# cvlab-stonybrook/s-volsdf

Measured on AMD Instinct MI355X. Metric: rendered rays/sec (1024-ray batch, 128 samples), higher is better.
Workload: dtype f32 (every product, forward and backward, as three fp16 MFMA products of two-piece fp16 operands with f32 accumulate; activation blocks hold both pieces: float32 accuracy class); 1 GPU; configs[1]: VolOpt.train_step (forward + MVS prior lookup + loss + backward + clip/guard/Adam), train mode, fast=1: 1024 rays/GPU x 128 coarse + 98 composited samples + 2048 eikonal points, 8x256 SDF MLP + 4x256 radiance MLP; mode=train, mlp_precision=fp16x2, launch=eager launches, rays_per_gpu=1024, rays_total=1024

## Files before the change

### include/svolsdf_hip.h

```cpp
#ifndef SVOLSDF_HIP_H
#define SVOLSDF_HIP_H

#include <stddef.h>
#include <stdint.h>

#ifdef __cplusplus
extern "C" {
#endif

int svs_version(void);
const char* svs_last_error_string(void);

int svs_set_deterministic(int on);
int svs_get_deterministic(void);

int svs_rays_from_uv(const float* uv, const float* pose, const float* intrinsics, int n_rays, float* ray_dirs,
                     float* cam_loc, float* depth_scale, void* hip_stream);

int svs_eikonal_points(const float* uniform_points, const float* cam_loc, const float* z_eik, const float* ray_dirs,
                       int n_rays, float* points, void* hip_stream);
int svs_stage_in(const void* pinned_host, void* device, size_t bytes, void* hip_stream);
int svs_split_last(const float* z, int n_rays, int n, float* head, float* last, void* hip_stream);

enum { SVS_MMA_F32 = 0, SVS_MMA_F16X2 = 1, SVS_MMA_F16X2_HALF = 2 };
// ... 55 lines not shown
                   const float* stream, int precision, float* abuf, float* sbar_out, float* absmax, void* hip_stream);
int svs_composite_bg(int n_rays, int n_samples, int n_bg, const float* z, const float* z_max, const float* sdf,
                     const float* rgb, const float* normals, const float* depth_scale, const float* beta_param,
                     float beta_min, const float* z_bg, const float* bg_out0, const float* bg_rgb, const float* bg_depth,
                     float* weights, float* bg_trans, float* bg_weights, float* rgb_values, float* depth_values,
                     float* depth_values_all, float* depth_vals, float* normal_map, void* hip_stream);
int svs_composite_bg_bwd(int n_rays, int n_samples, int n_bg, const float* z, const float* z_max, const float* sdf,
                         const float* rgb, const float* depth_scale, const float* beta_param, float beta_min,
                         const float* z_bg, const float* bg_out0, const float* bg_rgb, const float* d_rgb_values,
                         const float* d_weights, const float* d_depth_values, const float* d_depth_all,
                         const float* bg_depth, float* d_sdf, float* d_rgb,
                         float* d_bg_out0, float* d_bg_rgb, float* d_beta_ray, float* d_beta_param, void* hip_stream);

typedef struct svs_wgrad_job {
  const float *a0, *b0; long long sa0, sb0;
  const float *a1, *b1; long long sa1, sb1;
  const float* b_extra; long long s_extra;
  int n_points, ldw;
  float *dW, *db;
  const float* absmax;
  const float *rec0, *rec1;
} svs_wgrad_job;
int svs_wgrad_multi(const svs_wgrad_job* jobs, int n_jobs, int precision, void* hip_stream);
int svs_wgrad(const float* a0, const float* b0, long long sa0, long long sb0, const float* a1, const float* b1,
              long long sa1, long long sb1, const float* b_extra, long long s_extra, int n_points, int precision,
              const float* absmax, const float* rec0, const float* rec1, float* dW, int ldw, float* db, void* hip_stream);

size_t svs_block_bytes(int n_points, int blocks_per_tile);
size_t svs_rgb_zbuf_bytes(int n_points);
size_t svs_sdf_ubuf_bytes(int n_points);
size_t svs_sdf_gbuf_bytes(int n_points);
int svs_rgb_bwd(int n_points, const float* d_rgb, const float* rgb, const float* rbuf, const float* stream, int precision,
                float* zbuf, float* feat_bar, float* d_normals, float* absmax, void* hip_stream);
int svs_sdf_bwd_a(const float* points, int n_points, const float* cam, int cam_stride, const float* dirs, const float* z,
                  int S, int n_rays, const float* d_grad, const unsigned char* clamp_mask, const float* hbuf,
                  const float* gbuf, const float* stream, int precision, float* ubuf, float* a2buf, float* pebuf,
                  float* absmax, void* hip_stream);
int svs_sdf_bwd_b(int n_points, const float* d_sdf, const unsigned char* clamp_mask, const float* feat_bar,
                  int n_feat_points, const float* hbuf, const float* gbuf, const float* a2buf, const float* ubuf,
                  const float* stream, int precision, float* abuf, float* sbar_out, float* absmax, void* hip_stream);
int svs_lin8_row0_grad(const float* hbuf, const float* ubuf, const float* sbar, int n_points, int precision, float* out257,
                       void* hip_stream);
int svs_unpack_wgrad(const float* dWk, const float* dbk, int ldw, int map, int rows, int cols, int row_off,
                     const float* weight_v, const float* weight_g, const float* row0, float* grad_v, float* grad_g,
                     float* grad_b, void* hip_stream);
typedef struct svs_unpack_job {
// ... 255 lines not shown
```

### s-volsdf_amd/csrc/svs_wgrad.hip

```cpp
#include "svs_common.h"
#include "svs_mlp_layout.h"
#include "svs_ticket.h"
#include "svs_wgrad_maps.h"
#include <cstdlib>
#include <type_traits>

namespace svs {
namespace wgrad {

struct Pair {
  const float* a;
  const float* b;
  size_t stride_a, stride_b;
};

struct Args {
  Pair p[2];
  int n_pairs;
  int n_tiles;
  int n_valid_points;
  const float* b_extra;
  size_t stride_extra;
  float* dW;
  int ldw;
// ... 148 lines not shown
  __builtin_amdgcn_sched_barrier(0);
}
__device__ __forceinline__ unsigned lds_addr(const void* p) {
  return (unsigned)(unsigned long long)SVS_LDS(const void, p);
}

__device__ __forceinline__ void scale_from_absmax(const float* absmax, float& s, float& inv_s) {
  s = 1.0f; inv_s = 1.0f;
  if (!absmax) return;
  int e = (int)((__float_as_uint(*absmax) >> 23) & 0xff);
  e = e < 16 ? 16 : (e > 250 ? 250 : e);
  s = __uint_as_float((unsigned)(268 - e) << 23);
  inv_s = __uint_as_float((unsigned)(e - 14) << 23);
}

struct Job {
  Pair p[2];
  const float* rec[2];
  int n_pairs;
  int n_tiles;
  int n_valid_points;
  int b_tiles;
  int col0;
  float* dW;
  int ldw;
  float* db;
  const float* absmax;
  int wg_begin, wg_count;
  det::Ticket ticket;
};
constexpr int kMaxJobs = 20;
struct MultiArgs { Job job[kMaxJobs]; int n_jobs; int touch; int reverse; };
static_assert(sizeof(MultiArgs) <= 4096, "kernel arguments");

constexpr int kThreadsW = 512;
constexpr int kRT = 2, kCT = 16;
static_assert(maps::plane_reads_ok(kPlane), "transposed reads of the operand planes: bank conflict");
static_assert(maps::narrow_reads_ok(kExtraPiece), "transposed reads of the narrow B image: bank conflict");
static_assert(kPlane % 256 == 0 && kNarrowImg % 256 == 0 && kExtraPiece % 256 == 0 && Ring<true>::kSlotAll % 256 == 0 &&
              Ring<false>::kSlotAll % 256 == 0, "every region the reads are offset by starts on a 256-byte bank row");

typedef const __attribute__((address_space(1))) void* gvoid;

template <bool GP>
__global__ __launch_bounds__(kThreadsW, 1) void wgrad_h2_multi_kernel(MultiArgs ma) {
  typedef Ring<GP> R;
  constexpr int kSlot = R::kSlot, kSlotAll = R::kSlotAll, kRing = R::kRing, kAhead = R::kAhead, kB = R::kB;
  extern __shared__ __attribute__((aligned(16))) unsigned char smem_h2[];
  int jj = 0;
  for (int q = 1; q < ma.n_jobs; ++q) if ((int)blockIdx.x >= ma.job[q].wg_begin) jj = q;
  const Job& a = ma.job[jj];
  const int wg = (int)blockIdx.x - a.wg_begin, nwg = a.wg_count;
  const int tid = threadIdx.x, lane = tid & 63;
  const int wave = __builtin_amdgcn_readfirstlane(tid >> 6);
  const bool narrow = a.b_tiles == 1;
  float s_grad, inv_s;
  scale_from_absmax(a.absmax, s_grad, inv_s);

  f32x4 acc[kRT][kCT];
#pragma unroll
  for (int o = 0; o < kRT; ++o)
#pragma unroll
    for (int i = 0; i < kCT; ++i) acc[o][i] = (f32x4)(0.0f);
  float bsum[kRT];
#pragma unroll
  for (int o = 0; o < kRT; ++o) bsum[o] = 0.0f;

  unsigned char* ring = smem_h2;

  const int rg = lane >> 4;
  const int rd_even = maps::plane_base(0, lane), rd_odd = maps::plane_base(1, lane);
  const int a_off = 1024 * kRT * wave;
  const int rx = maps::narrow_base(lane);
  const int wp = lane & 31, whf = lane >> 5;
  const int wxoff = maps::narrow_at(8 * (wave & 3) + 4 * whf, wp);
  const int n_ct = narrow ? 2 : kCT;

  const bool two_pairs = a.n_pairs == 2;
  const int my_tiles = a.n_tiles > wg ? (a.n_tiles - 1 - wg) / nwg + 1 : 0;
  const int n_items = two_pairs ? 2 * my_tiles : my_tiles;
  const int n_valid = a.n_valid_points;
  const bool has_db = a.db != nullptr;
  const bool rev = ma.reverse != 0;
  const float* const pa0 = a.p[0].a; const float* const pb0 = a.p[0].b;
  const float* const pa1 = a.p[1].a; const float* const pb1 = a.p[1].b;
  const size_t sa0 = a.p[0].stride_a, sb0 = a.p[0].stride_b, sa1 = a.p[1].stride_a, sb1 = a.p[1].stride_b;
  const float* const rec0 = a.rec[0]; const float* const rec1 = a.rec[1];
  const bool has_scale = a.absmax != nullptr;
  auto tile_of = [&](int item) {
    const int k = two_pairs ? item >> 1 : item;
    return rev ? wg + (my_tiles - 1 - k) * nwg : wg + k * nwg;
  };

  auto issue = [&](int item) {
    const int t = tile_of(item), pi = two_pairs ? item & 1 : 0;
    const float* pa = (pi ? pa1 : pa0) + (size_t)t * (pi ? sa1 : sa0);
    const float* pb = (pi ? pb1 : pb0) + (size_t)t * (pi ? sb1 : sb0);
    unsigned char* slot = ring + (item % kRing) * kSlotAll;
#pragma unroll
    for (int j = 0; j < 2 * R::kPlanes; ++j) {
      const int piece = wave + 8 * j;
      __builtin_amdgcn_global_load_lds((gvoid)(reinterpret_cast<const f32x4*>(pa) + piece * 64 + lane),
                                       SVS_LDS(void, slot + piece * 1024), 16, 0, 0);
      if (!narrow)
        __builtin_amdgcn_global_load_lds((gvoid)(reinterpret_cast<const f32x4*>(pb) + piece * 64 + lane),
                                         SVS_LDS(void, slot + kB + piece * 1024), 16, 0, 0);
    }
    if (narrow)
      __builtin_amdgcn_global_load_lds((gvoid)(reinterpret_cast<const f32x4*>(pb) + (wave & 3) * 64 + lane),
                                       SVS_LDS(void, slot + kB + (wave & 3) * 1024), 16, 0, 0);
    if (has_scale)
      __builtin_amdgcn_global_load_lds((gvoid)((pi ? rec1 : rec0) + (size_t)t * 64 + lane),
                                       SVS_LDS(void, slot + kSlot + wave * 256), 4, 0, 0);
  };
  unsigned sink = 0;
  auto touch = [&](int item) {
    const int t = tile_of(item), pi = two_pairs ? item & 1 : 0;
    const Pair& p = a.p[pi];
    constexpr int kLines = R::kPlanes * (kPlane / 128);
    const int nb = narrow ? 32 : kLines;
    const float* q = tid < kLines ? p.a + (size_t)t * p.stride_a + tid * 32
                                  : p.b + (size_t)t * p.stride_b + (tid - kLines) * 32;
    if (tid < kLines + nb) asm volatile("global_load_dword %0, %1, off" : "+v"(sink) : "v"(q) : "memory");
  };
  const int ops = (narrow ? 2 * R::kPlanes + 1 : 4 * R::kPlanes) + (has_scale ? 1 : 0);

  auto stage_factors = [&](int item) {
// ... 50 lines not shown
  };
  for (int item = 0; item < n_items; ++item) {
    const int pi = two_pairs ? item & 1 : 0;
    const bool p0 = pi == 0;
    pre_stage(item);
    asm volatile("s_waitcnt lgkmcnt(0)\n\ts_barrier" ::: "memory");
    if (narrow) {
      stage_narrow(item);
      asm volatile("s_waitcnt lgkmcnt(0)\n\ts_barrier" ::: "memory");
    }
    auto issue_next = [&]() {
      if (item + kAhead < n_items) issue(item + kAhead);
      touched = false;
      if (touching && item + kAhead + 1 < n_items) { touch(item + kAhead + 1); touched = true; }
    };
    const unsigned la = lds_addr(ring + (item % kRing) * kSlotAll);
    const unsigned lb = la + kB;
    const unsigned ftab = la + kSlot + kRecBytes + wave * 64;
    const unsigned a_even = la + a_off + rd_even, a_odd = la + a_off + rd_odd;
    const unsigned b_even = lb + rd_even, b_odd = lb + rd_odd;
    const unsigned n_rd = lb + kNarrowImg + rx;
    const bool want_bias = has_db && p0;
    const bool two = narrow;
    Frag fa[kRT], fam[kRT];
    f32x4 fraw;
    static_for<kRT>([&](auto oc) {
      constexpr int o = decltype(oc)::value;
      tr_issue<1024 * o>(fa[o], o & 1 ? a_odd : a_even);
      if (GP) tr_issue<kPlane + 1024 * o>(fam[o], o & 1 ? a_odd : a_even);
    });
    lds_read128(fraw, ftab + 16 * rg);
    issue_next();
    lds_wait();
    f16x8 ah[kRT], am[kRT];
#pragma unroll
    for (int o = 0; o < kRT; ++o) {
      ah[o] = frag_of(fa[o]) * __builtin_bit_cast(f16x8, fraw);
      am[o] = GP ? frag_of(fam[o]) * __builtin_bit_cast(f16x8, fraw) : ah[o];
      if (want_bias) {
#pragma unroll
        for (int j = 0; j < 4; ++j) {
          const f16x2 h2v = {ah[o][2 * j], ah[o][2 * j + 1]};
          bsum[o] = __builtin_amdgcn_fdot2(h2v, one2, bsum[o], false);
          if (GP) {
            const f16x2 m2v = {am[o][2 * j], am[o][2 * j + 1]};
            bsum[o] = __builtin_amdgcn_fdot2(m2v, one2, bsum[o], false);
          }
        }
      }
    }
    static_for<kCT>([&](auto ic) {
      constexpr int i = decltype(ic)::value;
      if (i < n_ct) {
        Frag fh, fm;
        if (!narrow) {
          tr_issue<1024 * i>(fh, i & 1 ? b_odd : b_even);
          if (GP) tr_issue<kPlane + 1024 * i>(fm, i & 1 ? b_odd : b_even);
        } else if constexpr (i < 2) {
          tr_issue<1024 * i>(fh, n_rd);
          tr_issue<kExtraPiece + 1024 * i>(fm, n_rd);
        }
        lds_wait();
        const f16x8 bh = frag_of(fh), bm = frag_of(fm);
        if (two || GP) {
#pragma unroll
          for (int o = 0; o < kRT; ++o) acc[o][i] = __builtin_amdgcn_mfma_f32_16x16x32_f16(ah[o], bm, acc[o][i], 0, 0, 0);
        }
        if (GP) {
#pragma unroll
          for (int o = 0; o < kRT; ++o) acc[o][i] = __builtin_amdgcn_mfma_f32_16x16x32_f16(am[o], bh, acc[o][i], 0, 0, 0);
        }
#pragma unroll
        for (int o = 0; o < kRT; ++o) acc[o][i] = __builtin_amdgcn_mfma_f32_16x16x32_f16(ah[o], bh, acc[o][i], 0, 0, 0);
      }
    });
  }
  asm volatile("s_waitcnt vmcnt(0)" :: "v"(sink) : "memory");
  const int fcol = lane & 15;
  det::wait_turn(a.ticket, wg);
  static_for<kCT>([&](auto ic) {
    constexpr int i = decltype(ic)::value;
    const int c = a.col0 + 16 * i + fcol;
    if (i < n_ct && c < a.ldw) {
#pragma unroll
      for (int o = 0; o < kRT; ++o)
#pragma unroll
        for (int r = 0; r < 4; ++r)
          atomicAdd(&a.dW[(size_t)(16 * (kRT * wave + o) + 4 * rg + r) * a.ldw + c], acc[o][i][r] * inv_s);
    }
  });
  if (a.db) {
#pragma unroll
    for (int o = 0; o < kRT; ++o) {
      float sum = bsum[o];
      sum += __shfl_xor(sum, 16);
      sum += __shfl_xor(sum, 32);
      if (lane < 16) atomicAdd(&a.db[16 * (kRT * wave + o) + lane], sum * inv_s);
    }
  }
  det::pass_turn(a.ticket, wg);
}

}

}
}

using namespace svs;
using namespace svs::wgrad;
namespace h2 = svs::wgrad::h2;

extern "C" {

struct svs_wgrad_job {
  const float *a0, *b0; long long sa0, sb0;
  const float *a1, *b1; long long sa1, sb1;
  const float* b_extra; long long s_extra;
  int n_points, ldw;
  float *dW, *db;
  const float* absmax;
  const float *rec0, *rec1;
};

int svs_wgrad_multi(const svs_wgrad_job* jobs, int n_jobs, int precision, void* hip_stream) {
  if (!jobs || n_jobs < 1) { set_error("svs_wgrad_multi: no jobs"); return SVS_EINVAL; }
  int n_expanded = 0;
  for (int j = 0; j < n_jobs; ++j) n_expanded += jobs[j].b_extra ? 2 : 1;
  if (n_expanded > h2::kMaxJobs) { set_error("svs_wgrad_multi: at most %d jobs (b_extra counts twice)", h2::kMaxJobs); return SVS_EINVAL; }
  for (int j = 0; j < n_jobs; ++j) {
    const svs_wgrad_job& q = jobs[j];
    if (!q.a0 || !q.b0 || !q.dW || q.n_points <= 0 || q.ldw < 256 || q.ldw > 288 || (q.b_extra && q.ldw < 288) || (q.a1 && !q.b1)) {
      set_error("svs_wgrad_multi: bad argument in job %d", j); return SVS_EINVAL;
    }
    if (mlp::is_h2(precision) && q.absmax && (!q.rec0 || (q.a1 && !q.rec1))) {
      set_error("svs_wgrad_multi: job %d has absmax but no scale records", j); return SVS_EINVAL;
    }
  }
  hipStream_t s = (hipStream_t)hip_stream;
  if (mlp::is_h2(precision)) {
    const bool gp = precision == mlp::kFmtF16x2;
    h2::MultiArgs ma;
    int n = 0;
    long long work[h2::kMaxJobs], total = 0;
    for (int j = 0; j < n_jobs; ++j) {
      const svs_wgrad_job& q = jobs[j];
      h2::Job& J = ma.job[n];
      J.p[0] = Pair{q.a0, q.b0, (size_t)q.sa0, (size_t)q.sb0};
      J.rec[0] = q.rec0; J.rec[1] = q.rec1;
      J.n_pairs = 1;
      if (q.a1) { J.p[1] = Pair{q.a1, q.b1, (size_t)q.sa1, (size_t)q.sb1}; J.n_pairs = 2; }
      else { J.p[1] = J.p[0]; J.rec[1] = J.rec[0]; }
      J.n_tiles = (q.n_points + 31) / 32; J.n_valid_points = q.n_points;
      J.b_tiles = 8; J.col0 = 0; J.dW = q.dW; J.ldw = q.ldw; J.db = q.db; J.absmax = q.absmax;
      work[n] = (long long)J.n_tiles * J.n_pairs * 10;
      total += work[n++];
      if (q.b_extra) {
        h2::Job& X = ma.job[n];
        X = J;
        X.p[0].b = q.b_extra; X.p[0].stride_b = (size_t)q.s_extra; X.n_pairs = 1;
        X.b_tiles = 1; X.col0 = 256; X.db = nullptr;
        work[n] = (long long)X.n_tiles * 6;
        total += work[n++];
      }
    }
    ma.n_jobs = n;
    static const int touch_env = [] { const char* e = getenv("SVS_WGRAD_TOUCH"); return e ? atoi(e) : 0; }();
    ma.touch = touch_env;
    static const int reverse_env = [] { const char* e = getenv("SVS_WGRAD_REVERSE"); return e ? atoi(e) : 0; }();
    ma.reverse = reverse_env;
    (void)total;
    const int n_wg_total = 256;
    int count[h2::kMaxJobs];
    int used = 0;
    for (int j = 0; j < n; ++j) { count[j] = 1; ++used; }
    while (used < n_wg_total) {
      int best = -1;
      double load = 0.0;
      for (int j = 0; j < n; ++j) {
        if (count[j] >= ma.job[j].n_tiles) continue;
        const double l = (double)work[j] / count[j];
        if (l > load) { load = l; best = j; }
      }
      if (best < 0) break;
      ++count[best]; ++used;
    }
    int begin = 0;
    for (int j = 0; j < n; ++j) {
      ma.job[j].wg_begin = begin; ma.job[j].wg_count = count[j];
      begin += count[j];
      ma.job[j].ticket = det::Ticket{nullptr, 0u, 0u};
    }
    if (deterministic()) {
      int owner[h2::kMaxJobs], n_owner = 0;
      for (int j = 0; j < n; ++j) {
        owner[j] = -1;
        for (int k = 0; k < j; ++k)
          if (ma.job[k].dW == ma.job[j].dW && ma.job[k].col0 == ma.job[j].col0) { owner[j] = owner[k]; break; }
        if (owner[j] < 0) owner[j] = n_owner++;
      }
      unsigned* turn = det::take_slots((unsigned)n_owner);
      if (!turn) { set_error("svs_wgrad_multi: no turn counters (deterministic mode)"); return SVS_EINVAL; }
      unsigned total[h2::kMaxJobs] = {0};
      for (int j = 0; j < n; ++j) { ma.job[j].ticket.turn = turn + owner[j]; ma.job[j].ticket.first = total[owner[j]]; total[owner[j]] += (unsigned)count[j]; }
      for (int j = 0; j < n; ++j) ma.job[j].ticket.total = total[owner[j]];
    }
    static hipError_t e = hipFuncSetAttribute(reinterpret_cast<const void*>(h2::wgrad_h2_multi_kernel<false>),
                                              hipFuncAttributeMaxDynamicSharedMemorySize, h2::Ring<false>::kLdsBytes);
    static hipError_t ep = hipFuncSetAttribute(reinterpret_cast<const void*>(h2::wgrad_h2_multi_kernel<true>),
                                               hipFuncAttributeMaxDynamicSharedMemorySize, h2::Ring<true>::kLdsBytes);
    if (e != hipSuccess || ep != hipSuccess) {
      set_error("svs_wgrad_multi: hipFuncSetAttribute: %s", hipGetErrorString(e != hipSuccess ? e : ep)); return (int)(e != hipSuccess ? e : ep);
    }
    if (gp) h2::wgrad_h2_multi_kernel<true><<<begin, h2::kThreadsW, h2::Ring<true>::kLdsBytes, s>>>(ma);
    else h2::wgrad_h2_multi_kernel<false><<<begin, h2::kThreadsW, h2::Ring<false>::kLdsBytes, s>>>(ma);
    return check_launch("svs_wgrad_multi");
  }
  if (precision != mlp::kFmtF32) { set_error("svs_wgrad_multi: unknown precision %d", precision); return SVS_EINVAL; }
  for (int j = 0; j < n_jobs; ++j) {
    const svs_wgrad_job& q = jobs[j];
    Args a;
    a.p[0] = Pair{q.a0, q.b0, (size_t)q.sa0, (size_t)q.sb0};
    a.n_pairs = 1;
    if (q.a1) { a.p[1] = Pair{q.a1, q.b1, (size_t)q.sa1, (size_t)q.sb1}; a.n_pairs = 2; }
    a.n_tiles = (q.n_points + 31) / 32;
    a.n_valid_points = q.n_points;
    a.b_extra = q.b_extra; a.stride_extra = (size_t)q.s_extra;
    a.dW = q.dW; a.ldw = q.ldw; a.db = q.db;
    const int grid = a.n_tiles < 256 ? a.n_tiles : 256;
    a.ticket = det::Ticket{det::take_slots(1), 0u, (unsigned)grid};
    if (q.b_extra) {
      constexpr int lds = 2 * 32 * (260 + 292) * 4;
      static hipError_t e9 = hipFuncSetAttribute(reinterpret_cast<const void*>(wgrad_kernel<9>),
                                                 hipFuncAttributeMaxDynamicSharedMemorySize, lds);
      if (e9 != hipSuccess) { set_error("svs_wgrad_multi: hipFuncSetAttribute: %s", hipGetErrorString(e9)); return (int)e9; }
      wgrad_kernel<9><<<grid, 256, lds, s>>>(a);
    } else {
      constexpr int lds = 2 * 32 * (260 + 260) * 4;
// ... 19 lines not shown
```

### s-volsdf_amd/svs_hip/lib.py

```python
import ctypes
import os
from ctypes import POINTER, c_char_p, c_double, c_float, c_int, c_longlong, c_size_t, c_void_p

_HERE = os.path.dirname(os.path.abspath(__file__))
LIB_PATH = os.environ.get("SVS_LIB_PATH") or os.path.join(os.path.dirname(_HERE), "lib", "libsvolsdf_hip.so")

_lib = None


class SvsError(RuntimeError):
    pass


_P = c_void_p
_PP = POINTER(c_void_p)

class WGradJob(ctypes.Structure):
    _fields_ = [("a0", ctypes.c_void_p), ("b0", ctypes.c_void_p), ("sa0", ctypes.c_longlong), ("sb0", ctypes.c_longlong),
                ("a1", ctypes.c_void_p), ("b1", ctypes.c_void_p), ("sa1", ctypes.c_longlong), ("sb1", ctypes.c_longlong),
                ("b_extra", ctypes.c_void_p), ("s_extra", ctypes.c_longlong),
                ("n_points", ctypes.c_int), ("ldw", ctypes.c_int),
                ("dW", ctypes.c_void_p), ("db", ctypes.c_void_p), ("absmax", ctypes.c_void_p),
                ("rec0", ctypes.c_void_p), ("rec1", ctypes.c_void_p)]

# ... 27 lines not shown
    "svs_block_bytes": (c_size_t, [c_int, c_int]),
    "svs_rgb_zbuf_bytes": (c_size_t, [c_int]),
    "svs_sdf_ubuf_bytes": (c_size_t, [c_int]),
    "svs_rgb_bwd": (c_int, [c_int, _P, _P, _P, _P, c_int, _P, _P, _P, _P, _P]),
    "svs_sdf_bwd_a": (c_int, [_P, c_int, _P, c_int, _P, _P, c_int, c_int, _P, _P, _P, _P, _P, c_int, _P, _P, _P,
                              _P, _P]),
    "svs_sdf_bwd_b": (c_int, [c_int, _P, _P, _P, c_int, _P, _P, _P, _P, _P, c_int, _P, _P, _P, _P]),
    "svs_lin8_row0_grad": (c_int, [_P, _P, _P, c_int, c_int, _P, _P]),
    "svs_unpack_wgrad": (c_int, [_P, _P, c_int, c_int, c_int, c_int, c_int, _P, _P, _P, _P, _P, _P, _P]),
    "svs_unpack_wgrad_multi": (c_int, [_P, c_int, _P]),
    "svs_sampler_ctl_bytes": (c_size_t, [c_int, c_int]),
    "svs_sampler_ctl_stride": (c_int, []),
    "svs_sampler_cap": (c_int, []),
    "svs_sampler_max_new": (c_int, []),
    "svs_sampler_init": (c_int, [_P, c_int, _P, c_int, c_int, c_float, c_float, c_int, c_float, _P, c_float, c_int,
                                 _P, _P, _P, _P, c_int, _P, _P]),
    "svs_sampler_round": (c_int, [c_int, c_int, c_int, c_int, c_int, c_int, c_int, _P, c_float, c_float, c_int, c_float,
                                  c_float, _P, _P, _P, _P, _P, _P, _P, c_int, _P, _P, _P, _P, _P, _P, _P, _P, _P, _P]),
    "svs_composite": (c_int, [c_int, c_int, _P, _P, _P, _P, _P, _P, c_float, _P, _P, _P, _P, _P, _P]),
    "svs_composite_bwd": (c_int, [c_int, c_int, _P, _P, _P, _P, _P, c_float, _P, _P, _P, _P, _P, _P, _P, _P]),
    "svs_wgrad": (c_int, [_P, _P, ctypes.c_longlong, ctypes.c_longlong, _P, _P, ctypes.c_longlong, ctypes.c_longlong,
                          _P, ctypes.c_longlong, c_int, c_int, _P, _P, _P, _P, c_int, _P, _P]),
    "svs_wgrad_multi": (c_int, [_P, c_int, c_int, _P]),
    "svs_bg_points": (c_int, [_P, c_int, _P, c_int, c_int, _P, c_float, _P, _P, _P, _P]),
    "svs_bg_sdf_eval": (c_int, [_P, c_int, _P, c_int, _P, _P, _P, _P, _P, _P]),
    "svs_bg_rgb_bwd": (c_int, [c_int, _P, _P, _P, _P, c_int, _P, _P, _P, _P]),
    "svs_bg_sdf_bwd": (c_int, [c_int, _P, _P, _P, _P, _P, c_int, _P, _P, _P, _P]),
    "svs_bg_rbuf_bytes": (c_size_t, [c_int]),
    "svs_bg_rgb_eval": (c_int, [c_int, _P, c_int, _P, _P, c_int, _P, _P, _P]),
    "svs_composite_bg_bwd": (c_int, [c_int, c_int, c_int, _P, _P, _P, _P, _P, _P, c_float, _P, _P, _P, _P, _P, _P, _P, _P,
                                     _P, _P, _P, _P, _P, _P, _P]),
    "svs_composite_bg": (c_int, [c_int, c_int, c_int, _P, _P, _P, _P, _P, _P, _P, c_float, _P, _P, _P, _P,
                                 _P, _P, _P, _P, _P, _P, _P, _P, _P]),
    "svs_adam_workspace_bytes": (c_size_t, []),
    "svs_clip_guard_adam": (c_int, [_P, _P, _P, _P, ctypes.c_longlong, c_int, _P, c_double, c_double, c_double, c_double,
                                    c_double, _P, _P, _P]),
    "svs_cost_lookup": (c_int, [_P, _P, _P, _P, c_int, c_int, c_int, c_int, c_int, c_float, c_float, POINTER(c_float),
                                _PP, _PP, _PP, POINTER(c_int), _P, _P, _P, _P, _P]),
    "svs_loss": (c_int, [c_int, c_int, c_int, _P, _P, _P, _P, _P, _P, _P, c_float, c_float, c_float, c_float, c_float,
                         c_float, c_int, c_float, c_int, c_int, _P, _P, _P, _P, _P, _P, _P, _P]),
    "svs_loss_workspace_bytes": (c_size_t, [c_int, c_int]),
    "svs_conv2d": (c_int, [_P, _P, _P, _P, c_int, _P, c_int, c_int, c_int, c_int, c_int, c_int, c_int, _P]),
    "svs_featurenet_fpn_workspace_bytes": (c_size_t, [c_int, c_int, c_int]),
    "svs_featurenet_fpn": (c_int, [_P, c_int, c_int, c_int, _P, _P, _P, _P, _P, _P, _P]),
    "svs_featurenet_fpn2": (c_int, [_P, c_int, c_int, c_int, _P, _P, _P, _P, _P, _P, _P, _P]),
    "svs_conv2d_mfma_supported": (c_int, [c_int, c_int, c_int, c_int]),
# ... 183 lines not shown
```

### s-volsdf_amd/svs_hip/train.py

```python
import ctypes
import os

import torch

from . import lib as _lib
from .ops import _f32, _ptr, _ptr_array, _stream, default_precision, is_h2, F16X2, F16X2_HALF

KBLOCK = 128 * 64
KREC = 64


def block_stride(n_points):
    return ((n_points + 127) // 128) * 4 * KBLOCK
LDW = 288


def n_tiles_padded(n_points):
    return ((n_points + 127) // 128) * 4


def record_off(n_points, n_blocks, block):
    T = n_tiles_padded(n_points)
    return n_blocks * T * KBLOCK + block * T * KREC

# ... 31 lines not shown
        self.dWk = parts[0].view(slots, 256, LDW)
        self.dbk = parts[1].view(slots, 256)
        self.row0 = parts[2][:257]
        self.absmax = parts[3]

    def zero(self):
        self.flat.zero_()

    def bases(self):
        return self.dWk.data_ptr(), self.dbk.data_ptr(), self.absmax.data_ptr()


class _JobCache(dict):

    def memo(self, key, build):
        hit = self.get(key)
        if hit is None:
            if len(self) >= 64:
                self.clear()
            hit = self[key] = build()
        return hit


def _job_array(jobs):
    arr = (_lib.WGradJob * len(jobs))(*[_lib.WGradJob(*j) for j in jobs])
    return ctypes.cast(arr, ctypes.c_void_p), len(jobs), arr


def _f(addr, n_floats):
    return addr + 4 * n_floats


def wgrad_job(acc, slot, n_pts, amax, scaled, a0, sa0, b0, sb0, a1=None, sa1=0, b1=None, sb1=0, extra=None, sx=0,
              rec0=None, rec1=None):
    dWk, dbk, absmax = acc
    return (a0, b0, sa0, sb0, a1, b1, sa1, sb1, extra, sx, n_pts, LDW, _f(dWk, slot * 256 * LDW), _f(dbk, slot * 256),
            _f(absmax, amax) if scaled else None, rec0 if scaled else None, rec1 if scaled else None)


def rgb_wgrad_table(n_main, h2, acc, zbuf, feat, rbuf):
    LSm = block_stride(n_main)
    zrec = lambda l: _f(zbuf, record_off(n_main, 5, l))
    jobs = [wgrad_job(acc, 9, n_main, 1, h2, zbuf, KBLOCK, feat, KBLOCK, extra=_f(rbuf, 4 * LSm), sx=1024, rec0=zrec(0))]
    for l in range(1, 5):
        jobs.append(wgrad_job(acc, 9 + l, n_main, 1, h2, _f(zbuf, l * LSm), KBLOCK, _f(rbuf, (l - 1) * LSm), KBLOCK,
                              rec0=zrec(l)))
    return jobs


def sdf_wgrad_table(n_total, n_main, h2, acc, abuf, ubuf, pebuf, hbuf, gbuf, feat_bar):
    LS = block_stride(n_total)
    arec = lambda l: _f(abuf, record_off(n_total, 8, l))
    second = lambda l: dict(a1=_f(gbuf, l * LS), sa1=KBLOCK, b1=_f(ubuf, l * LS), sb1=KBLOCK,
                            rec1=_f(ubuf, record_off(n_total, 9, l)))
    jobs = [wgrad_job(acc, 0, n_total, 0, h2, abuf, KBLOCK, pebuf, KBLOCK, rec0=arec(0), **second(0))]
    for l in range(1, 8):
        jobs.append(wgrad_job(acc, l, n_total, 0, h2, _f(abuf, l * LS), KBLOCK, _f(hbuf, (l - 1) * LS), KBLOCK, rec0=arec(l),
                              **second(l)))
    jobs.append(wgrad_job(acc, 8, n_main, 2, h2, feat_bar, KBLOCK, _f(hbuf, 7 * LS), KBLOCK,
                          rec0=_f(feat_bar, record_off(n_main, 1, 0))))
    return jobs


BGRBUF = KBLOCK + 1024


def bg_wgrad_table(P, acc, abuf, zbuf, feat_bar, hbuf, pebuf, rbuf, feat):
    LS, Z2, T = block_stride(P), 2 * KBLOCK, n_tiles_padded(P)
    job = lambda slot, amax, *a, **k: wgrad_job(acc, slot, P, amax, True, *a, **k)
    arec = lambda l: _f(abuf, record_off(P, 8, l))
    jobs = [job(0, 0, abuf, KBLOCK, pebuf, KBLOCK, rec0=arec(0))]
    for l in range(1, 8):
        jobs.append(job(l, 0, _f(abuf, l * LS), KBLOCK, _f(hbuf, (l - 1) * LS), KBLOCK, rec0=arec(l)))
    jobs.append(job(8, 2, feat_bar, KBLOCK, _f(hbuf, 7 * LS), KBLOCK, rec0=_f(feat_bar, record_off(P, 1, 0))))
    zrec = lambda b: _f(zbuf, 2 * T * KBLOCK + b * T * KREC)
    jobs.append(job(9, 1, zbuf, Z2, feat, KBLOCK, rec0=zrec(0), extra=_f(rbuf, KBLOCK), sx=BGRBUF))
    jobs.append(job(10, 1, _f(zbuf, KBLOCK), Z2, rbuf, BGRBUF, rec0=zrec(1)))
    return jobs


def unpack_table(dWk, dbk, row0, layers, maps):
    jobs = []
    for net, l, slot, rows, cols, v, g, gv, gg, gb in layers:
        mp = maps[0] if (net == 0 and l == 4) else (maps[1] if (net == 1 and l == 0) else 0)
        last = net == 0 and l == 8
        jobs.append((_f(dWk, slot * 256 * LDW), _f(dbk, slot * 256), LDW, mp, rows, cols, 1 if last else 0, v, g,
                     row0 if last else None, gv, gg, gb))
    return jobs


def _unpack(accum, nets, maps, out, which=(0, 1)):
    dev = accum.dWk.device
    res, layers, keep = [], [], []
    for gi, (v, g, base) in enumerate(nets):
        group = []
        for l in range(len(v)) if gi in which else ():
            rows, cols = v[l].shape
            if out is not None:
                gv, gg, gb = out[gi][l]
            else:
                gv = torch.empty(rows, cols, device=dev)
# ... 48 lines not shown
        self._alloc(n_total, n_main)
        return self.d_sdf_full[:n_main].view(n_main, 1)

    def grad_extra_out(self, n_total, n_main):
        self._alloc(n_total, n_main)
        return self.d_grad_full[n_main:]

    def accumulate(self, keep, d_rgb, d_sdf, d_grad_extra, wait=True, side=True, defer_wgrad=False, extra=None):
        L = _lib.load()
        src = keep["src"]
        n_total, n_main = src.n, keep["rgb"].shape[0]
        if n_main % 32:
            raise NotImplementedError("rays*samples of a group must be a multiple of 32")
        self._alloc(n_total, n_main)
        dev, acc, S = self.dev, self.accum, self.streams
        hbuf, gbuf, mask = keep["hbuf"], keep["gbuf"], keep["clamp_mask"]
        rbuf, feat = keep["rbuf"], keep["feat_tiles"]

        prec = S.precision
        h2 = is_h2(prec)

        cache, bases = self._job_cache, acc.bases()

        def wgrad_multi(key, build, more):
            own = cache.memo(key, build)
            arr, n, _ = cache.memo(("arr",) + key + ((more["key"],) if more else ()),
                                   lambda: _job_array(own + (more["jobs"] if more else [])))
            _lib.check(L.svs_wgrad_multi(arr, n, prec, _stream()), "svs_wgrad_multi")

        d_rgb = _f32(d_rgb)
        d_grad = self.d_grad_full
        d_normals = d_grad[:n_main]
        n_extra = 0 if d_grad_extra is None else d_grad_extra.shape[0]
        if n_main + n_extra != n_total:
            raise ValueError("d_grad_extra must cover the points that follow the ray samples")
        if n_extra and d_grad_extra.data_ptr() != d_grad[n_main:].data_ptr():
            torch.mul(_f32(d_grad_extra), 1.0, out=d_grad[n_main:])
        _lib.check(L.svs_rgb_bwd(n_main, _ptr(d_rgb), _ptr(keep["rgb"]), _ptr(rbuf), _ptr(S.rgb), prec, _ptr(self.zbuf),
                                 _ptr(self.feat_bar), _ptr(d_normals), _ptr(acc.absmax) if h2 else None, _stream()),
                   "svs_rgb_bwd")
        if d_sdf is not None and d_sdf.data_ptr() == self.d_sdf_full.data_ptr() and d_sdf.numel() == n_main:
            d_sdf_full = self.d_sdf_full
        else:
            d_sdf_full = torch.zeros(n_total, device=dev)
            if d_sdf is not None:
                d_sdf_full[:n_main] = _f32(d_sdf).reshape(-1)
        main = torch.cuda.current_stream()
        if self._side is None:
            self._side = torch.cuda.Stream(device=dev)
        if os.environ.get("SVS_RGB_WGRAD_SIDE", "1") == "0":
            side = False
        side_stream = self._side if side else main
        rkey = ("rgb", n_main, prec, self.zbuf.data_ptr(), feat.data_ptr(), rbuf.data_ptr(), bases[0])
        rgb_jobs = lambda: rgb_wgrad_table(n_main, h2, bases, _ptr(self.zbuf), _ptr(feat), _ptr(rbuf))
        deferred = None
        if defer_wgrad:
            ev_rgb = torch.cuda.Event(); ev_rgb.record(main)
            deferred = dict(rgb=dict(jobs=cache.memo(rkey, rgb_jobs), key=rkey), ev_rgb=ev_rgb)
            join = None
        else:
            fork = torch.cuda.Event(); fork.record(main)
            with torch.cuda.stream(side_stream):
                if side:
                    side_stream.wait_event(fork)
                if extra is not None:
                    side_stream.wait_event(extra["ev_rgb"])
                wgrad_multi(rkey, rgb_jobs, extra["rgb"] if extra else None)
                join = torch.cuda.Event(); join.record(side_stream)
        st = _stream()
        _lib.check(L.svs_sdf_bwd_a(*src.args(), _ptr(d_grad), _ptr(mask), _ptr(hbuf), _ptr(gbuf), _ptr(S.sdf), prec,
                                   _ptr(self.ubuf), _ptr(self.a2buf), _ptr(self.pebuf),
                                   _ptr(acc.absmax) if h2 else None, st), "svs_sdf_bwd_a")
        _lib.check(L.svs_sdf_bwd_b(n_total, _ptr(d_sdf_full), _ptr(mask), _ptr(self.feat_bar), n_main, _ptr(hbuf),
                                   _ptr(gbuf), _ptr(self.a2buf), _ptr(self.ubuf), _ptr(S.sdf), prec, _ptr(self.abuf),
                                   _ptr(self.sbar), _ptr(acc.absmax) if h2 else None, st),
                   "svs_sdf_bwd_b")
        _lib.check(L.svs_lin8_row0_grad(_ptr(hbuf), _ptr(self.ubuf), _ptr(self.sbar), n_total, prec, _ptr(acc.row0),
                                        _stream()), "svs_lin8_row0_grad")
        ev = self.timer_events = ([torch.cuda.Event(enable_timing=True) for _ in range(2)] if self.time_wgrad else None)
        if ev:
            ev[0].record()
        skey = ("sdf", n_total, n_main, prec, self.abuf.data_ptr(), self.ubuf.data_ptr(), self.pebuf.data_ptr(),
                hbuf.data_ptr(), gbuf.data_ptr(), self.feat_bar.data_ptr(), bases[0])
        sdf_jobs = lambda: sdf_wgrad_table(n_total, n_main, h2, bases, _ptr(self.abuf), _ptr(self.ubuf), _ptr(self.pebuf),
                                           _ptr(hbuf), _ptr(gbuf), _ptr(self.feat_bar))
        if defer_wgrad:
            deferred["sdf"] = dict(jobs=cache.memo(skey, sdf_jobs), key=skey)
            deferred["ev_all"] = torch.cuda.Event(); deferred["ev_all"].record(main)
            deferred["hold"] = self._hold = (d_grad, d_sdf_full, d_normals, d_rgb)
            return deferred
        if extra is not None:
            main.wait_event(extra["ev_all"])
        wgrad_multi(skey, sdf_jobs, extra["sdf"] if extra else None)
        if ev:
            ev[1].record()
        if wait and side:
            main.wait_event(join)
        self._hold = (d_grad, d_sdf_full, d_normals, d_rgb)
        return join

    def run(self, sdf_params, rgb_params, keep, d_rgb, d_sdf, d_grad_extra, out=None):
        self.streams.pack(sdf_params, rgb_params)
        self.accum.zero()
        self.accumulate(keep, d_rgb, d_sdf, d_grad_extra)
        return finalize(self.accum, sdf_params, rgb_params, out)


class BgBackward:
    def __init__(self, device, precision=None):
        L = _lib.load()
        self.dev = device
        self.precision = default_precision() if precision is None else int(precision)
        self.sdf_stream = torch.empty(L.svs_stream_bytes(6) // 4, device=device)
        self.rgb_stream = torch.empty(L.svs_stream_bytes(8) // 4, device=device)
        self.ws = torch.empty(L.svs_pack_workspace_bytes() // 4, device=device)
        self.accum = WGradAccum(device, slots=11)
# ... 19 lines not shown
            return cur[1:]
        L = _lib.load()
        z = lambda nbytes: torch.zeros(nbytes // 4, device=self.dev)
        cur = (n, z(L.svs_block_bytes(n, 2)),
               z(L.svs_block_bytes(n, 1)), z(L.svs_block_bytes(n, 8)), z(L.svs_block_bytes(n, 1) // (128 * 2)))
        self._scratch[slot] = cur
        return cur[1:]

    def accumulate(self, keep, d_bg_rgb, d_bg_out0, slot=0):
        L = _lib.load()
        P = keep["bg_rgb"].shape[0]
        zbuf, feat_bar, abuf, sbar = self._alloc(P, slot)
        st = _stream()
        hbuf, ghat7, pebuf, rbuf, feat = keep["bg_hbuf"], keep["bg_ghat7"], keep["bg_pebuf"], keep["bg_rbuf"], keep["bg_feat"]
        d_bg_rgb, d_bg_out0 = _f32(d_bg_rgb), _f32(d_bg_out0)
        prec = self.precision
        _lib.check(L.svs_bg_rgb_bwd(P, _ptr(d_bg_rgb), _ptr(keep["bg_rgb"]), _ptr(rbuf), _ptr(self.rgb_stream), prec, _ptr(zbuf),
                                    _ptr(feat_bar), _ptr(self.absmax), st), "svs_bg_rgb_bwd")
        _lib.check(L.svs_bg_sdf_bwd(P, _ptr(d_bg_out0), _ptr(feat_bar), _ptr(hbuf), _ptr(ghat7), _ptr(self.sdf_stream), prec,
                                    _ptr(abuf), _ptr(sbar), _ptr(self.absmax), st), "svs_bg_sdf_bwd")
        _lib.check(L.svs_lin8_row0_grad(_ptr(hbuf), None, _ptr(sbar), P, prec, _ptr(self.row0), st), "svs_lin8_row0_grad")
        ptrs = tuple(_ptr(t) for t in (abuf, zbuf, feat_bar, hbuf, pebuf, rbuf, feat))
        bases = self.accum.bases()
        arr, n, _ = self._job_cache.memo(("bg", P, prec) + ptrs + bases[:1],
                                         lambda: _job_array(bg_wgrad_table(P, bases, *ptrs)))
        _lib.check(L.svs_wgrad_multi(arr, n, prec, st), "svs_wgrad_multi(bg)")
        self._hold = getattr(self, "_hold", {})
        self._hold[slot] = (d_bg_rgb, d_bg_out0)

    def finalize(self, sdf_wb, rgb_wb, out=None):
        if out is not None:
            out = [[(gw, None, gb) for gw, gb in group] for group in out]
        res = _unpack(self.accum, ((sdf_wb[0], None, 0), (rgb_wb[0], None, 9)), (3, 4), out)
        return tuple([(gw, gb) for gw, _, gb in group] for group in res)


def algorithmic_bytes_per_point(precision=None):
    precision = default_precision() if precision is None else precision
    if is_h2(precision):
        half = 512 if precision == F16X2_HALF else 1024
        pair = 1024
        return {"svs_sdf_bwd_a": 8 * half + 9 * half + pair,
                "svs_sdf_bwd_b": 8 * half + 8 * half + 8 * half + half + 8 * half,
                "wgrad_sdf": 8 * (half + half + half + half) + half + half,
                "wgrad_radiance": 5 * half + 4 * half + half + 128,
                "svs_lin8_row0_grad": pair + half,
                "svs_sdf_outputs": 8 * pair + 8 * pair + 8 * half + pair}
    blk = 1024
    return {"svs_sdf_bwd_a": (8 + 8 + 9 + 8 + 1) * blk, "svs_sdf_bwd_b": (8 + 8 + 1 + 1 + 8) * blk,
# ... 3 lines not shown
```

Baseline: 295,000 rays/s.

## Skip dead row and column pieces in fp16x2 weight-gradient kernel

Adds a per-job live-row extent (A and B piece counts) staged through a new host call, with a templated kernel variant. For jobs with narrow layers (the last z-bar layer with 3 rows, positional encodings with 39/84 rows), waves whose row pieces are dead skip their LDS loads, MFMAs and atomics, and tiles beyond the live B columns are dropped. Only the background wgrad path stages extents by default; the foreground path is gated off. This trades extra kernel instantiations, register pressure and a host call for less wasted MFMA and load work on padded rows.

Result: no change. 292,600 rays/s (-0.8%).

```diff
diff --git a/include/svolsdf_hip.h b/include/svolsdf_hip.h
--- a/include/svolsdf_hip.h
+++ b/include/svolsdf_hip.h
@@ -101,6 +101,7 @@
   const float *rec0, *rec1;
 } svs_wgrad_job;
 int svs_wgrad_multi(const svs_wgrad_job* jobs, int n_jobs, int precision, void* hip_stream);
+int svs_wgrad_live_rows(const int* a_rows, const int* b_rows, int n_jobs);
 int svs_wgrad(const float* a0, const float* b0, long long sa0, long long sb0, const float* a1, const float* b1,
               long long sa1, long long sb1, const float* b_extra, long long s_extra, int n_points, int precision,
               const float* absmax, const float* rec0, const float* rec1, float* dW, int ldw, float* db, void* hip_stream);
diff --git a/s-volsdf_amd/csrc/svs_wgrad.hip b/s-volsdf_amd/csrc/svs_wgrad.hip
--- a/s-volsdf_amd/csrc/svs_wgrad.hip
+++ b/s-volsdf_amd/csrc/svs_wgrad.hip
@@ -194,6 +194,7 @@
   int n_valid_points;
   int b_tiles;
   int col0;
+  int a_pieces, b_pieces;
   float* dW;
   int ldw;
   float* db;
@@ -214,13 +215,11 @@
 
 typedef const __attribute__((address_space(1))) void* gvoid;
 
-template <bool GP>
-__global__ __launch_bounds__(kThreadsW, 1) void wgrad_h2_multi_kernel(MultiArgs ma) {
+template <bool GP, bool WHOLE>
+__device__ __forceinline__ void wgrad_h2_body(const MultiArgs& ma, const int jj) {
   typedef Ring<GP> R;
   constexpr int kSlot = R::kSlot, kSlotAll = R::kSlotAll, kRing = R::kRing, kAhead = R::kAhead, kB = R::kB;
   extern __shared__ __attribute__((aligned(16))) unsigned char smem_h2[];
-  int jj = 0;
-  for (int q = 1; q < ma.n_jobs; ++q) if ((int)blockIdx.x >= ma.job[q].wg_begin) jj = q;
   const Job& a = ma.job[jj];
   const int wg = (int)blockIdx.x - a.wg_begin, nwg = a.wg_count;
   const int tid = threadIdx.x, lane = tid & 63;
@@ -246,7 +245,11 @@
   const int rx = maps::narrow_base(lane);
   const int wp = lane & 31, whf = lane >> 5;
   const int wxoff = maps::narrow_at(8 * (wave & 3) + 4 * whf, wp);
-  const int n_ct = narrow ? 2 : kCT;
+  const int a_pieces = WHOLE ? kCT : __builtin_amdgcn_readfirstlane(a.a_pieces);
+  const int b_pieces = WHOLE ? kCT : __builtin_amdgcn_readfirstlane(a.b_pieces);
+  const int n_ct = narrow ? 2 : b_pieces;
+  const int n_rt = WHOLE ? kRT : (a_pieces - kRT * wave < 0 ? 0 : (a_pieces - kRT * wave > kRT ? kRT : a_pieces - kRT * wave));
+  const int n_ct_w = n_rt > 0 ? n_ct : 0;
 
   const bool two_pairs = a.n_pairs == 2;
   const int my_tiles = a.n_tiles > wg ? (a.n_tiles - 1 - wg) / nwg + 1 : 0;
@@ -271,10 +274,11 @@
     unsigned char* slot = ring + (item % kRing) * kSlotAll;
 #pragma unroll
     for (int j = 0; j < 2 * R::kPlanes; ++j) {
-      const int piece = wave + 8 * j;
-      __builtin_amdgcn_global_load_lds((gvoid)(reinterpret_cast<const f32x4*>(pa) + piece * 64 + lane),
-                                       SVS_LDS(void, slot + piece * 1024), 16, 0, 0);
-      if (!narrow)
+      const int piece = wave + 8 * j, in_plane = wave + 8 * (j & 1);
+      if (!GP || in_plane < a_pieces)
+        __builtin_amdgcn_global_load_lds((gvoid)(reinterpret_cast<const f32x4*>(pa) + piece * 64 + lane),
+                                         SVS_LDS(void, slot + piece * 1024), 16, 0, 0);
+      if (!narrow && (!GP || in_plane < b_pieces))
         __builtin_amdgcn_global_load_lds((gvoid)(reinterpret_cast<const f32x4*>(pb) + piece * 64 + lane),
                                          SVS_LDS(void, slot + kB + piece * 1024), 16, 0, 0);
     }
@@ -371,19 +375,23 @@
     const unsigned n_rd = lb + kNarrowImg + rx;
     const bool want_bias = has_db && p0;
     const bool two = narrow;
+    const bool r0 = WHOLE || n_rt > 0, r1 = WHOLE || n_rt > 1;
     Frag fa[kRT], fam[kRT];
     f32x4 fraw;
     static_for<kRT>([&](auto oc) {
       constexpr int o = decltype(oc)::value;
-      tr_issue<1024 * o>(fa[o], o & 1 ? a_odd : a_even);
-      if (GP) tr_issue<kPlane + 1024 * o>(fam[o], o & 1 ? a_odd : a_even);
+      if (o == 0 ? r0 : r1) {
+        tr_issue<1024 * o>(fa[o], o & 1 ? a_odd : a_even);
+        if (GP) tr_issue<kPlane + 1024 * o>(fam[o], o & 1 ? a_odd : a_even);
+      }
     });
-    lds_read128(fraw, ftab + 16 * rg);
+    if (r0) lds_read128(fraw, ftab + 16 * rg);
     issue_next();
     lds_wait();
     f16x8 ah[kRT], am[kRT];
 #pragma unroll
     for (int o = 0; o < kRT; ++o) {
+      if (o == 0 ? !r0 : !r1) { ah[o] = (f16x8)(_Float16)0.0f; am[o] = ah[o]; continue; }
       ah[o] = frag_of(fa[o]) * __builtin_bit_cast(f16x8, fraw);
       am[o] = GP ? frag_of(fam[o]) * __builtin_bit_cast(f16x8, fraw) : ah[o];
       if (want_bias) {
@@ -398,29 +406,32 @@
         }
       }
     }
+    auto tile = [&](auto ic, auto nr_c) {
+      constexpr int i = decltype(ic)::value, NR = decltype(nr_c)::value;
+      Frag fh, fm;
+      if (!narrow) {
+        tr_issue<1024 * i>(fh, i & 1 ? b_odd : b_even);
+        if (GP) tr_issue<kPlane + 1024 * i>(fm, i & 1 ? b_odd : b_even);
+      } else if constexpr (i < 2) {
+        tr_issue<1024 * i>(fh, n_rd);
+        tr_issue<kExtraPiece + 1024 * i>(fm, n_rd);
+      }
+      lds_wait();
+      const f16x8 bh = frag_of(fh), bm = frag_of(fm);
+      if (two || GP) {
+#pragma unroll
+        for (int o = 0; o < NR; ++o) acc[o][i] = __builtin_amdgcn_mfma_f32_16x16x32_f16(ah[o], bm, acc[o][i], 0, 0, 0);
+      }
+      if (GP) {
+#pragma unroll
+        for (int o = 0; o < NR; ++o) acc[o][i] = __builtin_amdgcn_mfma_f32_16x16x32_f16(am[o], bh, acc[o][i], 0, 0, 0);
+      }
+#pragma unroll
+      for (int o = 0; o < NR; ++o) acc[o][i] = __builtin_amdgcn_mfma_f32_16x16x32_f16(ah[o], bh, acc[o][i], 0, 0, 0);
+    };
     static_for<kCT>([&](auto ic) {
-      constexpr int i = decltype(ic)::value;
-      if (i < n_ct) {
-        Frag fh, fm;
-        if (!narrow) {
-          tr_issue<1024 * i>(fh, i & 1 ? b_odd : b_even);
-          if (GP) tr_issue<kPlane + 1024 * i>(fm, i & 1 ? b_odd : b_even);
-        } else if constexpr (i < 2) {
-          tr_issue<1024 * i>(fh, n_rd);
-          tr_issue<kExtraPiece + 1024 * i>(fm, n_rd);
-        }
-        lds_wait();
-        const f16x8 bh = frag_of(fh), bm = frag_of(fm);
-        if (two || GP) {
-#pragma unroll
-          for (int o = 0; o < kRT; ++o) acc[o][i] = __builtin_amdgcn_mfma_f32_16x16x32_f16(ah[o], bm, acc[o][i], 0, 0, 0);
-        }
-        if (GP) {
-#pragma unroll
-          for (int o = 0; o < kRT; ++o) acc[o][i] = __builtin_amdgcn_mfma_f32_16x16x32_f16(am[o], bh, acc[o][i], 0, 0, 0);
-        }
-#pragma unroll
-        for (int o = 0; o < kRT; ++o) acc[o][i] = __builtin_amdgcn_mfma_f32_16x16x32_f16(ah[o], bh, acc[o][i], 0, 0, 0);
+      if (decltype(ic)::value < n_ct_w) {
+        if (WHOLE || r1) tile(ic, std::integral_constant<int, kRT>{}); else tile(ic, std::integral_constant<int, 1>{});
       }
     });
   }
@@ -430,17 +441,20 @@
   static_for<kCT>([&](auto ic) {
     constexpr int i = decltype(ic)::value;
     const int c = a.col0 + 16 * i + fcol;
-    if (i < n_ct && c < a.ldw) {
+    if (i < n_ct_w && c < a.ldw) {
 #pragma unroll
       for (int o = 0; o < kRT; ++o)
-#pragma unroll
-        for (int r = 0; r < 4; ++r)
-          atomicAdd(&a.dW[(size_t)(16 * (kRT * wave + o) + 4 * rg + r) * a.ldw + c], acc[o][i][r] * inv_s);
+        if (o < n_rt) {
+#pragma unroll
+          for (int r = 0; r < 4; ++r)
+            atomicAdd(&a.dW[(size_t)(16 * (kRT * wave + o) + 4 * rg + r) * a.ldw + c], acc[o][i][r] * inv_s);
+        }
     }
   });
   if (a.db) {
 #pragma unroll
     for (int o = 0; o < kRT; ++o) {
+      if (o >= n_rt) continue;
       float sum = bsum[o];
       sum += __shfl_xor(sum, 16);
       sum += __shfl_xor(sum, 32);
@@ -450,6 +464,14 @@
   det::pass_turn(a.ticket, wg);
 }
 
+template <bool GP, bool LIVE>
+__global__ __launch_bounds__(kThreadsW, 1) void wgrad_h2_multi_kernel(MultiArgs ma) {
+  int jj = 0;
+  for (int q = 1; q < ma.n_jobs; ++q) if ((int)blockIdx.x >= ma.job[q].wg_begin) jj = q;
+  if (!LIVE || (ma.job[jj].a_pieces == kCT && ma.job[jj].b_pieces == kCT)) wgrad_h2_body<GP, true>(ma, jj);
+  else wgrad_h2_body<GP, false>(ma, jj);
+}
+
 }
 
 }
@@ -459,7 +481,26 @@
 using namespace svs::wgrad;
 namespace h2 = svs::wgrad::h2;
 
+namespace {
+struct LiveRows { int n; int a[h2::kMaxJobs], b[h2::kMaxJobs]; };
+thread_local LiveRows g_live = {-1, {0}, {0}};
+int live_pieces(int rows) { return rows <= 0 || rows >= 256 ? 16 : (rows + 15) / 16; }
+}
+
 extern "C" {
+
+int svs_wgrad_live_rows(const int* a_rows, const int* b_rows, int n_jobs) {
+  g_live.n = -1;
+  if (!a_rows || !b_rows || n_jobs < 1 || n_jobs > h2::kMaxJobs) {
+    set_error("svs_wgrad_live_rows: needs a_rows, b_rows and 1..%d jobs", h2::kMaxJobs); return SVS_EINVAL;
+  }
+  for (int j = 0; j < n_jobs; ++j) {
+    if (a_rows[j] < 0 || b_rows[j] < 0) { set_error("svs_wgrad_live_rows: negative count in job %d", j); return SVS_EINVAL; }
+    g_live.a[j] = a_rows[j]; g_live.b[j] = b_rows[j];
+  }
+  g_live.n = n_jobs;
+  return SVS_OK;
+}
 
 struct svs_wgrad_job {
   const float *a0, *b0; long long sa0, sb0;
@@ -472,6 +513,11 @@
 };
 
 int svs_wgrad_multi(const svs_wgrad_job* jobs, int n_jobs, int precision, void* hip_stream) {
+  const LiveRows live = g_live;
+  g_live.n = -1;
+  if (live.n >= 0 && live.n != n_jobs) {
+    set_error("svs_wgrad_multi: live extents staged for %d jobs, called with %d", live.n, n_jobs); return SVS_EINVAL;
+  }
   if (!jobs || n_jobs < 1) { set_error("svs_wgrad_multi: no jobs"); return SVS_EINVAL; }
   int n_expanded = 0;
   for (int j = 0; j < n_jobs; ++j) n_expanded += jobs[j].b_extra ? 2 : 1;
@@ -501,13 +547,15 @@
       else { J.p[1] = J.p[0]; J.rec[1] = J.rec[0]; }
       J.n_tiles = (q.n_points + 31) / 32; J.n_valid_points = q.n_points;
       J.b_tiles = 8; J.col0 = 0; J.dW = q.dW; J.ldw = q.ldw; J.db = q.db; J.absmax = q.absmax;
+      J.a_pieces = live.n >= 0 ? live_pieces(live.a[j]) : 16;
+      J.b_pieces = live.n >= 0 ? live_pieces(live.b[j]) : 16;
       work[n] = (long long)J.n_tiles * J.n_pairs * 10;
       total += work[n++];
       if (q.b_extra) {
         h2::Job& X = ma.job[n];
         X = J;
         X.p[0].b = q.b_extra; X.p[0].stride_b = (size_t)q.s_extra; X.n_pairs = 1;
-        X.b_tiles = 1; X.col0 = 256; X.db = nullptr;
+        X.b_tiles = 1; X.col0 = 256; X.db = nullptr; X.b_pieces = 16;
         work[n] = (long long)X.n_tiles * 6;
         total += work[n++];
       }
@@ -553,15 +601,23 @@
       for (int j = 0; j < n; ++j) { ma.job[j].ticket.turn = turn + owner[j]; ma.job[j].ticket.first = total[owner[j]]; total[owner[j]] += (unsigned)count[j]; }
       for (int j = 0; j < n; ++j) ma.job[j].ticket.total = total[owner[j]];
     }
-    static hipError_t e = hipFuncSetAttribute(reinterpret_cast<const void*>(h2::wgrad_h2_multi_kernel<false>),
-                                              hipFuncAttributeMaxDynamicSharedMemorySize, h2::Ring<false>::kLdsBytes);
-    static hipError_t ep = hipFuncSetAttribute(reinterpret_cast<const void*>(h2::wgrad_h2_multi_kernel<true>),
-                                               hipFuncAttributeMaxDynamicSharedMemorySize, h2::Ring<true>::kLdsBytes);
-    if (e != hipSuccess || ep != hipSuccess) {
-      set_error("svs_wgrad_multi: hipFuncSetAttribute: %s", hipGetErrorString(e != hipSuccess ? e : ep)); return (int)(e != hipSuccess ? e : ep);
-    }
-    if (gp) h2::wgrad_h2_multi_kernel<true><<<begin, h2::kThreadsW, h2::Ring<true>::kLdsBytes, s>>>(ma);
-    else h2::wgrad_h2_multi_kernel<false><<<begin, h2::kThreadsW, h2::Ring<false>::kLdsBytes, s>>>(ma);
+    bool any_live = false;
+    for (int j = 0; j < n; ++j) any_live = any_live || ma.job[j].a_pieces < h2::kCT || ma.job[j].b_pieces < h2::kCT;
+    static const hipError_t e = [] {
+      hipError_t r = hipSuccess;
+      const void* k[4] = {reinterpret_cast<const void*>(h2::wgrad_h2_multi_kernel<false, false>),
+                          reinterpret_cast<const void*>(h2::wgrad_h2_multi_kernel<false, true>),
+                          reinterpret_cast<const void*>(h2::wgrad_h2_multi_kernel<true, false>),
+                          reinterpret_cast<const void*>(h2::wgrad_h2_multi_kernel<true, true>)};
+      for (int i = 0; i < 4 && r == hipSuccess; ++i)
+        r = hipFuncSetAttribute(k[i], hipFuncAttributeMaxDynamicSharedMemorySize, i < 2 ? h2::Ring<false>::kLdsBytes : h2::Ring<true>::kLdsBytes);
+      return r;
+    }();
+    if (e != hipSuccess) { set_error("svs_wgrad_multi: hipFuncSetAttribute: %s", hipGetErrorString(e)); return (int)e; }
+    if (gp && any_live) h2::wgrad_h2_multi_kernel<true, true><<<begin, h2::kThreadsW, h2::Ring<true>::kLdsBytes, s>>>(ma);
+    else if (gp) h2::wgrad_h2_multi_kernel<true, false><<<begin, h2::kThreadsW, h2::Ring<true>::kLdsBytes, s>>>(ma);
+    else if (any_live) h2::wgrad_h2_multi_kernel<false, true><<<begin, h2::kThreadsW, h2::Ring<false>::kLdsBytes, s>>>(ma);
+    else h2::wgrad_h2_multi_kernel<false, false><<<begin, h2::kThreadsW, h2::Ring<false>::kLdsBytes, s>>>(ma);
     return check_launch("svs_wgrad_multi");
   }
   if (precision != mlp::kFmtF32) { set_error("svs_wgrad_multi: unknown precision %d", precision); return SVS_EINVAL; }
diff --git a/s-volsdf_amd/svs_hip/lib.py b/s-volsdf_amd/svs_hip/lib.py
--- a/s-volsdf_amd/svs_hip/lib.py
+++ b/s-volsdf_amd/svs_hip/lib.py
@@ -73,6 +73,7 @@
     "svs_wgrad": (c_int, [_P, _P, ctypes.c_longlong, ctypes.c_longlong, _P, _P, ctypes.c_longlong, ctypes.c_longlong,
                           _P, ctypes.c_longlong, c_int, c_int, _P, _P, _P, _P, c_int, _P, _P]),
     "svs_wgrad_multi": (c_int, [_P, c_int, c_int, _P]),
+    "svs_wgrad_live_rows": (c_int, [_P, _P, c_int]),
     "svs_bg_points": (c_int, [_P, c_int, _P, c_int, c_int, _P, c_float, _P, _P, _P, _P]),
     "svs_bg_sdf_eval": (c_int, [_P, c_int, _P, c_int, _P, _P, _P, _P, _P, _P]),
     "svs_bg_rgb_bwd": (c_int, [c_int, _P, _P, _P, _P, c_int, _P, _P, _P, _P]),
diff --git a/s-volsdf_amd/svs_hip/train.py b/s-volsdf_amd/svs_hip/train.py
--- a/s-volsdf_amd/svs_hip/train.py
+++ b/s-volsdf_amd/svs_hip/train.py
@@ -77,9 +77,26 @@
         return hit
 
 
-def _job_array(jobs):
+def _job_array(jobs, live=None):
     arr = (_lib.WGradJob * len(jobs))(*[_lib.WGradJob(*j) for j in jobs])
-    return ctypes.cast(arr, ctypes.c_void_p), len(jobs), arr
+    ext = None
+    if live is not None:
+        a_rows, b_rows = live
+        if not len(a_rows) == len(b_rows) == len(jobs):
+            raise ValueError("live extents must name every job")
+        keep = ((ctypes.c_int * len(jobs))(*a_rows), (ctypes.c_int * len(jobs))(*b_rows))
+        ext = (ctypes.cast(keep[0], ctypes.c_void_p), ctypes.cast(keep[1], ctypes.c_void_p), keep)
+    return ctypes.cast(arr, ctypes.c_void_p), len(jobs), arr, ext
+
+
+def _wgrad_launch(L, arr, n, ext, prec, stream, what):
+    if ext is not None and L.svs_wgrad_live_rows(ext[0], ext[1], n):
+        _lib.check(-1, "svs_wgrad_live_rows")
+    _lib.check(L.svs_wgrad_multi(arr, n, prec, stream), what)
+
+
+ZBAR_LAST_ROWS, PE_ROWS, BG_PE_ROWS = 3, 39, 84
+STAGE_LIVE_FOREGROUND, STAGE_LIVE_BACKGROUND = False, True
 
 
 def _f(addr, n_floats):
@@ -101,6 +118,10 @@
         jobs.append(wgrad_job(acc, 9 + l, n_main, 1, h2, _f(zbuf, l * LSm), KBLOCK, _f(rbuf, (l - 1) * LSm), KBLOCK,
                               rec0=zrec(l)))
     return jobs
+
+
+def rgb_wgrad_live():
+    return [0, 0, 0, 0, ZBAR_LAST_ROWS], [0, 0, 0, 0, 0]
 
 
 def sdf_wgrad_table(n_total, n_main, h2, acc, abuf, ubuf, pebuf, hbuf, gbuf, feat_bar):
@@ -117,6 +138,10 @@
     return jobs
 
 
+def sdf_wgrad_live():
+    return [0] * 9, [PE_ROWS] + [0] * 8
+
+
 BGRBUF = KBLOCK + 1024
 
 
@@ -132,6 +157,10 @@
     jobs.append(job(9, 1, zbuf, Z2, feat, KBLOCK, rec0=zrec(0), extra=_f(rbuf, KBLOCK), sx=BGRBUF))
     jobs.append(job(10, 1, _f(zbuf, KBLOCK), Z2, rbuf, BGRBUF, rec0=zrec(1)))
     return jobs
+
+
+def bg_wgrad_live():
+    return [0] * 10 + [ZBAR_LAST_ROWS], [BG_PE_ROWS] + [0] * 10
 
 
 def unpack_table(dWk, dbk, row0, layers, maps):
@@ -226,11 +255,12 @@
 
         cache, bases = self._job_cache, acc.bases()
 
-        def wgrad_multi(key, build, more):
+        def wgrad_multi(key, build, live, more):
             own = cache.memo(key, build)
-            arr, n, _ = cache.memo(("arr",) + key + ((more["key"],) if more else ()),
-                                   lambda: _job_array(own + (more["jobs"] if more else [])))
-            _lib.check(L.svs_wgrad_multi(arr, n, prec, _stream()), "svs_wgrad_multi")
+            both = lambda: (tuple(x + y for x, y in zip(live, more["live"])) if more else live) if STAGE_LIVE_FOREGROUND else None
+            arr, n, _, ext = cache.memo(("arr",) + key + ((more["key"],) if more else ()),
+                                        lambda: _job_array(own + (more["jobs"] if more else []), both()))
+            _wgrad_launch(L, arr, n, ext, prec, _stream(), "svs_wgrad_multi")
 
         d_rgb = _f32(d_rgb)
         d_grad = self.d_grad_full
@@ -260,7 +290,7 @@
         deferred = None
         if defer_wgrad:
             ev_rgb = torch.cuda.Event(); ev_rgb.record(main)
-            deferred = dict(rgb=dict(jobs=cache.memo(rkey, rgb_jobs), key=rkey), ev_rgb=ev_rgb)
+            deferred = dict(rgb=dict(jobs=cache.memo(rkey, rgb_jobs), key=rkey, live=rgb_wgrad_live()), ev_rgb=ev_rgb)
             join = None
         else:
             fork = torch.cuda.Event(); fork.record(main)
@@ -269,7 +299,7 @@
                     side_stream.wait_event(fork)
                 if extra is not None:
                     side_stream.wait_event(extra["ev_rgb"])
-                wgrad_multi(rkey, rgb_jobs, extra["rgb"] if extra else None)
+                wgrad_multi(rkey, rgb_jobs, rgb_wgrad_live(), extra["rgb"] if extra else None)
                 join = torch.cuda.Event(); join.record(side_stream)
         st = _stream()
         _lib.check(L.svs_sdf_bwd_a(*src.args(), _ptr(d_grad), _ptr(mask), _ptr(hbuf), _ptr(gbuf), _ptr(S.sdf), prec,
@@ -289,13 +319,13 @@
         sdf_jobs = lambda: sdf_wgrad_table(n_total, n_main, h2, bases, _ptr(self.abuf), _ptr(self.ubuf), _ptr(self.pebuf),
                                            _ptr(hbuf), _ptr(gbuf), _ptr(self.feat_bar))
         if defer_wgrad:
-            deferred["sdf"] = dict(jobs=cache.memo(skey, sdf_jobs), key=skey)
+            deferred["sdf"] = dict(jobs=cache.memo(skey, sdf_jobs), key=skey, live=sdf_wgrad_live())
             deferred["ev_all"] = torch.cuda.Event(); deferred["ev_all"].record(main)
             deferred["hold"] = self._hold = (d_grad, d_sdf_full, d_normals, d_rgb)
             return deferred
         if extra is not None:
             main.wait_event(extra["ev_all"])
-        wgrad_multi(skey, sdf_jobs, extra["sdf"] if extra else None)
+        wgrad_multi(skey, sdf_jobs, sdf_wgrad_live(), extra["sdf"] if extra else None)
         if ev:
             ev[1].record()
         if wait and side:
@@ -361,9 +391,10 @@
         _lib.check(L.svs_lin8_row0_grad(_ptr(hbuf), None, _ptr(sbar), P, prec, _ptr(self.row0), st), "svs_lin8_row0_grad")
         ptrs = tuple(_ptr(t) for t in (abuf, zbuf, feat_bar, hbuf, pebuf, rbuf, feat))
         bases = self.accum.bases()
-        arr, n, _ = self._job_cache.memo(("bg", P, prec) + ptrs + bases[:1],
-                                         lambda: _job_array(bg_wgrad_table(P, bases, *ptrs)))
-        _lib.check(L.svs_wgrad_multi(arr, n, prec, st), "svs_wgrad_multi(bg)")
+        arr, n, _, ext = self._job_cache.memo(("bg", P, prec) + ptrs + bases[:1],
+                                              lambda: _job_array(bg_wgrad_table(P, bases, *ptrs),
+                                                                 bg_wgrad_live() if STAGE_LIVE_BACKGROUND else None))
+        _wgrad_launch(L, arr, n, ext, prec, st, "svs_wgrad_multi(bg)")
         self._hold = getattr(self, "_hold", {})
         self._hold[slot] = (d_bg_rgb, d_bg_out0)
 
```
